# mims-harvard/GNNDelete

Measured on AMD Instinct MI355X. Metric: Del-op train iters/sec, higher is better.
Workload: dtype f32; 1 GPU; synth-collab GCN 2-layer, 5.0% IN edge deletion, full-graph Del step (both_layerwise, mse_mean); num_nodes=235868, in_dim=128, hidden_dim=128, out_dim=64, train_edges_undirected=2122296, df_edges=53057, sdf_edges=1602188, spmm_nnz=1838056, S1=178921, S2=188697, hip_graph=True, matrix_products=fp32 matrix instruction (v_mfma_f32_32x32x2_f32), parallelism=single, ranks_seen=1

## Files before the change

gnndelete_amd/_lib.py:

```python
import ctypes
import os
import re

_HERE = os.path.dirname(os.path.abspath(__file__))
LIB_PATH = os.environ.get('GNNDELETE_HIP_LIB') or os.path.join(_HERE, 'lib', 'libgnndelete_hip.so')
HEADER_PATH = os.path.join(os.path.dirname(_HERE), 'include', 'gnndelete_hip.h')

_i32, _i64, _f32, _f64, _p = ctypes.c_int32, ctypes.c_int64, ctypes.c_float, ctypes.c_double, ctypes.c_void_p

ABI_VERSION = 9

PROTOTYPES = {
    'gd_abi_version': (ctypes.c_int, []),
    'gd_last_error_string': (ctypes.c_char_p, []),
    'gd_build_source_hash': (ctypes.c_char_p, []),
    'gd_matrix_split': (ctypes.c_int, []),
    'gd_set_matrix_split': (ctypes.c_int, [ctypes.c_int]),
    'gd_csr_from_coo_workspace': (_i64, [_i32, _i64]),
    'gd_csr_from_coo': (ctypes.c_int, [_p, _p, _i64, _i32, _p, _p, _p, _p, _p, _i64, _p]),
    'gd_gcn_norm_f32': (ctypes.c_int, [_p, _p, _i32, _p, _p]),
    'gd_spmm_csr_f32': (ctypes.c_int, [_p, _p, _p, _p, _i64, _p, _i64, _p, _f32, _i32, _i32, _p]),
    'gd_spmm_csr_balanced_f32': (ctypes.c_int, [_p, _i32, _p, _i32, _p, _p, _p, _i64, _p, _i64, _p, _f32, _p, _p, _i32,
                                                _i32, _i32, _p, _p]),
    'gd_spmm_csr_onepass_f32': (ctypes.c_int, [_p, _i32, _p, _p, _p, _i64, _p, _i64, _p, _f32, _p, _i32, _i32, _i32, _p, _p]),
    'gd_spmm_csr_onepass_wide_f32': (ctypes.c_int, [_p, _i32, _p, _p, _p, _i64, _p, _i64, _p, _f32, _p, _i32, _i32, _i32, _p, _p]),
    'gd_rows_gemm_wgrad_reduce_f32': (ctypes.c_int, [_p, _i32, _i32, _i32, _p, _i32, _p, _p, _p, _p, _f64, _f64, _f64, _f64, _p]),
    'gd_step_tail_f32': (ctypes.c_int, [_p, _i32, _i32, _i32, _p, _p, _p, _p, _p, _i32, _i32, _i32, _p, _p, _p, _p, _f64, _f64, _f64, _f64,
                                        _p, _i32, _p, _i32, _p, _i32, _p, _p, _p, _p]),
    'gd_step_tail_parts_f32': (ctypes.c_int, [_p, _i32, _i32, _i32, _p, _p, _p, _p, _p, _i32, _i32, _i32, _p, _p, _p, _p, _f64, _f64, _f64, _f64,
                                        _p, _i32, _p, _i32, _p, _i32, _p, _p, _p, _p]),
    'gd_rgcn_conv_f32': (ctypes.c_int, [_p, _p, _p, _p, _p, _p, _i64, _i32, _p, _i32, _i32, _p, _i64, _i32, _i32, _p]),
    'gd_rowpair_loss_f32': (ctypes.c_int, [_i32, _p, _i64, _p, _p, _i64, _p, _i32, _i32, _p, _p, _i64, _p]),
    'gd_random_walk': (ctypes.c_int, [_p, _p, _i32, _p, _i32, _i32, ctypes.c_uint64, _p, _p]),
    'gd_negative_edges': (ctypes.c_int, [_p, _i64, _i64, ctypes.c_uint64, _p, _i64, _p, _i64, _p]),
    'gd_rank_counts_f32': (ctypes.c_int, [_p, _i64, _p, _i64, _p, _p, _p]),
    'gd_subset_rank_workspace': (_i64, [_i64, _i64]),
    'gd_subset_rank_metrics': (ctypes.c_int, [_p, _p, _p, _p, _p, _i64, _i64, _i64, _i64, _i64, _p, _p, _p, _i64, _p]),
    'gd_subset_rank_metrics_drawn': (ctypes.c_int, [_p, _p, _p, _p, ctypes.c_uint64, ctypes.c_uint64, _i64, _i64, _i64, _i64, _p, _p, _p, _i64, _p]),
    'gd_subset_draw': (ctypes.c_int, [ctypes.c_uint64, ctypes.c_uint64, _i64, _i64, _i64, _p, _i64, _p]),
    'gd_rgcn_tile_kl': (ctypes.c_int32, [_i32, _i32, _i32, _i32]),
    'gd_rgcn_pack_weight_f32': (ctypes.c_int, [_p, _i32, _i32, _i32, _i32, _i32, _p, _p]),
    'gd_rgcn_wave_covers': (ctypes.c_int32, [_i32, _i32, _i32]),
    'gd_rgcn_wave_conv_f32': (ctypes.c_int, [_p, _i32, _i32, _p, _i32, _p, _p, _p, _p, _i64, _i32, _p, _i32, _p, _i64, _i32, _i32, _i32, _p]),
    'gd_rgcn_tile_conv_f32': (ctypes.c_int, [_p, _p, _p, _p, _p, _p, _p, _i32, _p, _i64, _i32, _p, _i32, _i32, _p, _i64, _i32,
                                             _i32, _p, _p, _i32, _p, _p]),
    'gd_rgcn_mean_f32': (ctypes.c_int, [_p, _p, _p, _i64, _p, _i64, _i32, _i32, _i32, _p]),
    'gd_gat_aggregate_f32': (ctypes.c_int, [_p, _p, _p, _p, _p, _i64, _p, _i64, _p, _p, _f32, _i32, _i32, _p]),
    'gd_gat_aggregate_bwd_f32': (ctypes.c_int, [_p, _p, _p, _p, _p, _p, _p, _p, _p, _i64, _p, _i64, _p, _i64,
                                                _p, _p, _p, _f32, _i32, _i32, _p]),
    'gd_gat_balanced_scratch': (_i64, [_i32, _i32]),
    'gd_gat_aggregate_balanced_f32': (ctypes.c_int, [_p, _i32, _p, _i32, _i32, _p, _p, _p, _p, _i64, _p, _i64, _p, _p, _p,
                                                     _p, _f32, _i32, _i32, _i32, _p]),
    'gd_gat_edge_grads_balanced_f32': (ctypes.c_int, [_p, _i32, _p, _i32, _p, _p, _p, _p, _p, _p, _i64, _p, _i64, _p,
                                                      _p, _p, _p, _f32, _i32, _i32, _p, _p]),
    'gd_row_dots_f32': (ctypes.c_int, [_p, _i64, _i32, _i32, _p, _p, _p, _p, _p]),
    'gd_gat_transpose_edges_f32': (ctypes.c_int, [_p, _p, _p, _i32, _p, _p, _p]),
    'gd_rank1_add2_f32': (ctypes.c_int, [_p, _i64, _i32, _i32, _p, _p, _p, _p, _p]),
    'gd_segment_sum_f32': (ctypes.c_int, [_p, _p, _p, _i32, _p, _p]),
# ... 166 lines not shown
```

gnndelete_amd/csrc/spmm.hip:

```cpp
#include <stdlib.h>
#include <string.h>

#include "common.h"
#include "tail_jobs.h"

namespace gd {

template <int LPR, int VPL, bool MEAN>
__global__ __launch_bounds__(256) void spmm_vec_kernel(const int32_t* __restrict__ rowptr,
                                                       const int32_t* __restrict__ col,
                                                       const float* __restrict__ val,
                                                       const float* __restrict__ x, int64_t ldx,
                                                       float* __restrict__ y, int64_t ldy,
                                                       const float* __restrict__ bias, float self_coef,
                                                       int32_t n_rows, int32_t x_rows_mod, int32_t d4) {
  constexpr int G = kWave / LPR;
  const int lane = threadIdx.x & 63;
  const int row = blockIdx.x * 4 + (threadIdx.x >> 6);
  if (row >= n_rows) return;
  const int g = lane / LPR;
  const int li = lane % LPR;
  const int start = rowptr[row];
  const int end = rowptr[row + 1];

// ... 482 lines not shown
          acc = f4_fma(wj[2], xv[2], f4_fma(wj[1], xv[1], f4_fma(wj[0], xv[0], acc)));
        }
        base += kWave;
        if (base >= d0.z) break;
        const int k2 = min(base + lane, nnz - 1);
        c_cur = colt[k2];
        w_raw = val ? val[k2] : 1.0f;
      }
      acc = f4_group_sum<16>(acc);
      const int wave = threadIdx.x >> 6;
      if (g == 0) grp_red[wave][li] = acc;
      __syncthreads();
      if (wave == 0 && g == 0) {
        float4 o = f4_add(f4_add(f4_add(grp_red[0][li], grp_red[1][li]), grp_red[2][li]), grp_red[3][li]);
        if (self_coef != 0.0f)
          o = f4_fma(self_coef, *reinterpret_cast<const float4*>(reinterpret_cast<const char*>(xs) + (__umul24((uint32_t)row, pitch_b) + lo)), o);
        if (bias) o = f4_add(o, bias_s[li]);
        *reinterpret_cast<float4*>(reinterpret_cast<char*>(y) + (__umul24((uint32_t)row, pitch_y) + lo)) = o;
      }
      __syncthreads();
    }
    d0 = d1;
    d1 = d2;
  }
}

__global__ __launch_bounds__(256) __attribute__((amdgpu_waves_per_eu(8, 8))) void spmm_wide_kernel(
    const int4* __restrict__ items, int32_t n_items, const int32_t* __restrict__ xcd_bounds, const int32_t* __restrict__ colt,
    const float* __restrict__ val, const float* __restrict__ x, int64_t ldx, float* __restrict__ y, int64_t ldy,
    const float* __restrict__ bias, float self_coef, const float* __restrict__ xs, int32_t nnz) {
  spmm_wide_body(items, n_items, xcd_bounds, colt, val, x, ldx, y, ldy, bias, self_coef, xs, nnz, blockIdx.x, gridDim.x);
}

__global__ __launch_bounds__(256) __attribute__((amdgpu_waves_per_eu(8, 8))) void spmm_wide_hosted_kernel(
    const int4* __restrict__ items, int32_t n_items, const int32_t* __restrict__ xcd_bounds, const int32_t* __restrict__ colt,
    const float* __restrict__ val, const float* __restrict__ x, int64_t ldx, float* __restrict__ y, int64_t ldy,
    const float* __restrict__ bias, float self_coef, const float* __restrict__ xs, int32_t nnz, TailHost host) {
  if (blockIdx.x < (uint32_t)host.nh) {
    tail_host_block(host, (int)blockIdx.x);
    return;
  }
  spmm_wide_body(items, n_items, xcd_bounds, colt, val, x, ldx, y, ldy, bias, self_coef, xs, nnz, blockIdx.x - host.nh, gridDim.x - host.nh);
}

__global__ __launch_bounds__(256) void spmm_fixup_kernel(const int4* __restrict__ split, int32_t n_split,
                                                         const float* __restrict__ scratch,
                                                         const float* __restrict__ x, int64_t ldx,
                                                         float* __restrict__ y, int64_t ldy,
                                                         const float* __restrict__ bias, float self_coef,
                                                         int32_t d4) {
  const int lane = threadIdx.x & 63;
  const int i = blockIdx.x * 4 + (threadIdx.x >> 6);
  if (i >= n_split) return;
  const int4 sp = split[i];
  const int row = sp.x, slot0 = sp.y, n = sp.z;
  for (int vec = lane; vec < d4; vec += kWave) {
    float4 o = f4_zero();
    const float4* sp4 = reinterpret_cast<const float4*>(scratch + (int64_t)slot0 * d4 * 4) + vec;
    int s = 0;
    for (; s + 4 <= n; s += 4) {
      const float4 p0 = sp4[(int64_t)s * d4], p1 = sp4[(int64_t)(s + 1) * d4], p2 = sp4[(int64_t)(s + 2) * d4],
                   p3 = sp4[(int64_t)(s + 3) * d4];
      o = f4_add(f4_add(f4_add(f4_add(o, p0), p1), p2), p3);
    }
    for (; s < n; ++s) o = f4_add(o, sp4[(int64_t)s * d4]);
    if (self_coef != 0.0f) o = f4_fma(self_coef, reinterpret_cast<const float4*>(x + (int64_t)row * ldx)[vec], o);
// ... 186 lines not shown
  const float* xs = x_self ? x_self : x;
  GD_REQUIRE(aligned16(xs) && xs != y, GD_E_ALIGN, "gd_spmm_csr_balanced_f32: bad x_self");
  float* scratch_arg = scratch ? scratch : reinterpret_cast<float*>(const_cast<int32_t*>(items));
  int rc = launch_persist(items, n_items, col, val, x, ldx, y, ldy, bias, self_coef, xs, scratch_arg, d, nnz, x_rows,
                          xcd_bounds, s);
  if (rc || n_split == 0) return rc;
  hipLaunchKernelGGL(spmm_fixup_kernel, dim3((n_split + 3) / 4), dim3(256), 0, s, reinterpret_cast<const int4*>(split),
                     n_split, scratch, xs, ldx, y, ldy, bias, self_coef, d4);
  return launched("spmm_fixup");
}

extern "C" int gd_spmm_csr_onepass_f32(const int32_t* items, int32_t n_items, const int32_t* col, const float* val,
                                       const float* x, int64_t ldx, float* y, int64_t ldy, const float* bias,
                                       float self_coef, const float* x_self, int32_t d, int32_t nnz, int32_t x_rows,
                                       const int32_t* xcd_bounds, void* stream) {
  using namespace gd;
  GD_REQUIRE(col && x && y && xcd_bounds && (items || n_items == 0), GD_E_NULL, "gd_spmm_csr_onepass_f32: null pointer");
  GD_REQUIRE(n_items >= 0 && n_items % 4 == 0 && d > 0 && d % 4 == 0 && d <= 1024 && ldx % 4 == 0 && ldy % 4 == 0, GD_E_DIM,
             "gd_spmm_csr_onepass_f32: d=%d must be a multiple of 4 (<=1024) with 16-byte row strides, n_items a multiple of 4", d);
  GD_REQUIRE(aligned16(x) && aligned16(y) && aligned16(items) && (!bias || aligned16(bias)), GD_E_ALIGN,
             "gd_spmm_csr_onepass_f32: unaligned pointer");
  GD_REQUIRE(x != y, GD_E_DIM, "gd_spmm_csr_onepass_f32: x and y must not alias");
  if (n_items == 0) return GD_OK;
  GD_REQUIRE(nnz > 0, GD_E_DIM, "gd_spmm_csr_onepass_f32: items over an index array without entries (nnz=%d)", nnz);
  const float* xs = x_self ? x_self : x;
  GD_REQUIRE(aligned16(xs) && xs != y, GD_E_ALIGN, "gd_spmm_csr_onepass_f32: bad x_self");
  return launch_persist(items, n_items, col, val, x, ldx, y, ldy, bias, self_coef, xs, nullptr, d, nnz, x_rows,
                        xcd_bounds, (hipStream_t)stream);
}

namespace gd {
static int launch_wide(const char* name, const int32_t* items, int32_t n_items, const int32_t* col_tagged, const float* val, const float* x,
                       int64_t ldx, float* y, int64_t ldy, const float* bias, float self_coef, const float* x_self, int32_t d,
                       int32_t nnz, int32_t x_rows, const int32_t* xcd_bounds, const TailHost* host, void* stream) {
  GD_REQUIRE(col_tagged && x && y && xcd_bounds && (items || n_items == 0), GD_E_NULL, "%s: null pointer", name);
  GD_REQUIRE(n_items >= 0 && n_items % 4 == 0 && d == 64 && ldx % 4 == 0 && ldy % 4 == 0 && ldx >= d && ldy >= d, GD_E_DIM,
             "%s: d must be 64 (got %d) with 16-byte row strides, n_items a multiple of 4", name, d);
  GD_REQUIRE(aligned16(x) && aligned16(y) && aligned16(items) && (!bias || aligned16(bias)), GD_E_ALIGN, "%s: unaligned pointer", name);
  GD_REQUIRE(x != y, GD_E_DIM, "%s: x and y must not alias", name);
  GD_REQUIRE(x_rows > 0 && x_rows < (1 << 24) && ldx * 4 < (1 << 24) && ldy * 4 < (1 << 24) &&
                 (int64_t)x_rows * ldx * 4 < (1ll << 32) && (int64_t)x_rows * ldy * 4 < (1ll << 32), GD_E_DIM,
             "%s: x and y must be smaller than 4 GiB with row ids and pitches below 2^24", name);
  GD_REQUIRE(!host || n_items > 0, GD_E_DIM, "%s: the tail's jobs need a launch to ride on (n_items = 0)", name);
  if (n_items == 0) return GD_OK;
  GD_REQUIRE(nnz > 0, GD_E_DIM, "%s: items over an index array without entries (nnz=%d)", name, nnz);
  const float* xs = x_self ? x_self : x;
  GD_REQUIRE(aligned16(xs) && xs != y, GD_E_ALIGN, "%s: bad x_self", name);
  const char* e = getenv("GD_SPMM_GRID_CAP");
  const int cap_env = e ? atoi(e) : 0;
  const int cap = cap_env > 0 ? cap_env : GD_SPMM_WIDE_GRID_CAP;
  int nblk = (n_items + 3) / 4;
  if (nblk > cap) nblk = cap;
  nblk = (nblk + 7) / 8 * 8;
  if (host) {
    hipLaunchKernelGGL(spmm_wide_hosted_kernel, dim3(host->nh + nblk), dim3(256), 0, (hipStream_t)stream,
                       reinterpret_cast<const int4*>(items), n_items, xcd_bounds, col_tagged, val, x, ldx, y, ldy, bias, self_coef, xs, nnz,
                       *host);
    return launched("spmm_wide_hosted");
  }
  hipLaunchKernelGGL(spmm_wide_kernel, dim3(nblk), dim3(256), 0, (hipStream_t)stream, reinterpret_cast<const int4*>(items), n_items,
                     xcd_bounds, col_tagged, val, x, ldx, y, ldy, bias, self_coef, xs, nnz);
  return launched("spmm_wide");
}
}

extern "C" int gd_spmm_csr_onepass_wide_f32(const int32_t* items, int32_t n_items, const int32_t* col_tagged, const float* val,
                                            const float* x, int64_t ldx, float* y, int64_t ldy, const float* bias,
                                            float self_coef, const float* x_self, int32_t d, int32_t nnz, int32_t x_rows,
                                            const int32_t* xcd_bounds, void* stream) {
  return gd::launch_wide("gd_spmm_csr_onepass_wide_f32", items, n_items, col_tagged, val, x, ldx, y, ldy, bias, self_coef, x_self, d, nnz,
                         x_rows, xcd_bounds, nullptr, stream);
}

extern "C" int gd_spmm_csr_onepass_wide_hosted_f32(
    const int32_t* items, int32_t n_items, const int32_t* col_tagged, const float* val, const float* x, int64_t ldx, float* y, int64_t ldy,
    const float* bias, float self_coef, const float* x_self, int32_t d, int32_t nnz, int32_t x_rows, const int32_t* xcd_bounds,
    const float* partials1_t, const float* colsum1, int32_t n_part1, int32_t d1, const float* w1, const float* w1_t, const float* b1,
    float* dw1, float* param1, float* exp_avg1, float* exp_avg_sq1, float* w_fold, float* bias_fold, const float* partials2,
    int32_t n_part2, int32_t d2, int32_t accumulate2, float* dw2, float* param2, float* exp_avg2, float* exp_avg_sq2, double lr,
    double beta1, double beta2, double eps, const float* loss_partials1, int32_t n1, const float* loss_partials2, int32_t n2, float* hist,
    int32_t capacity, int32_t* pos, int32_t* iter, int32_t* arrive, void* stream) {
  using namespace gd;
  const char* name = "gd_spmm_csr_onepass_wide_hosted_f32";
  GD_REQUIRE(n_part1 >= 0 && n_part2 >= 0 && n_part1 + n_part2 > 0, GD_E_DIM,
             "%s: a hosted launch carries job 1, job 2 or both (partial counts %d, %d)", name, n_part1, n_part2);
  GD_REQUIRE(iter, GD_E_NULL, "%s: null iteration counter", name);
  TailHost h{};
  h.lr = lr; h.beta1 = beta1; h.beta2 = beta2; h.eps = eps;
  h.fin = TailFin{loss_partials1, n1, loss_partials2, n2, hist, capacity, pos, iter, arrive};
  if (n_part1 > 0) {
    GD_REQUIRE(partials1_t && colsum1 && w1 && w1_t && b1 && dw1 && param1 && exp_avg1 && exp_avg_sq1 && w_fold && bias_fold, GD_E_NULL,
               "%s: null pointer of job 1", name);
    GD_REQUIRE(d1 == 128, GD_E_DIM, "%s: the folded layer-1 job is 128 wide (d1=%d)", name, d1);
    GD_REQUIRE(aligned16(partials1_t), GD_E_ALIGN, "%s: unaligned partials of job 1", name);
    h.j1 = TailJob{partials1_t, n_part1, d1 * d1, 0, dw1, param1, exp_avg1, exp_avg_sq1};
    h.fo = TailFold1{colsum1, w1, b1, w_fold, bias_fold};
    h.w1t = w1_t;
    h.n1b = 128;
  }
  if (n_part2 > 0) {
    GD_REQUIRE(partials2 && dw2 && param2 && exp_avg2 && exp_avg_sq2, GD_E_NULL, "%s: null pointer of job 2", name);
    GD_REQUIRE(hist && pos && arrive && capacity > 0 && n1 >= 0 && n2 >= 0 && (n1 == 0 || loss_partials1) && (n2 == 0 || loss_partials2),
               GD_E_NULL, "%s: null bookkeeping pointer", name);
    GD_REQUIRE(d2 > 0 && d2 % 4 == 0 && d2 <= 128, GD_E_DIM, "%s: d2=%d must be a multiple of 4, at most 128", name, d2);
// ... 39 lines not shown
```

gnndelete_amd/engine.py:

```python
import os
import warnings
from typing import NamedTuple

import torch

from . import _lib, ops
from ._lib import check, ptr, stream_ptr
from .capture import capture_iterations
from .graph import graph_for
from .nn import GATConv, GCNConv, GINConv, RGCNConv, SAGEConv

LOSS_TYPES = ('both_all', 'both_layerwise', 'only2_layerwise', 'only2_all', 'only1')


class StepFacts(NamedTuple):
    mode: str
    loss_type: str
    family: str
    h: int
    o: int
    s1: int
    s2: int
    folded1: bool
    n_rows1: int
# ... 663 lines not shown
        if idx is not None or self._mfma_weight(weight):
            return ops.rows_gemm(x, idx, weight, trans_w=True, const_w=True, relu_in=relu_in, out=out)
        if ops.mfma_out_width(out_f):
            xin = torch.relu(x) if relu_in else x
            return ops.gemm_wide(xin, ops._const_weight(weight, True)[0], const_x=not relu_in, const_w=True)
        if in_f <= 1024:
            return ops.rows_gemm(x, None, weight, trans_w=True, const_w=True, relu_in=relu_in)
        raise NotImplementedError(f'NodeembEngine: a {in_f} -> {out_f} Linear has no kernel (inputs above 1,024 floats need an output '
                                  'width in {32, 64, 96, 128}); there is no vendor-BLAS fallback')

    def _linear_relu_z1(self, weight, idx=None, out=None):
        if not self._split1:
            return self._linear(self.z1, weight, relu_in=True, idx=idx, out=out)
        if self._chain_expl:
            assert idx is None
            return ops.rows_gemm_select_chain(self._a1, self._idx1c, self._w1, self._b1, self.pre1, self.z1, self.idx1, weight, out=out)
        if idx is not None or self._mfma_weight(weight):
            return ops.rows_gemm_select(self.pre1, self.z1, self._sel1, weight, trans_w=True, const_w=True, relu_in=True,
                                        out=out, idx=idx)
        z = torch.where(self._sel1.bool()[:, None], self.z1, self.pre1)
        return self._linear(z, weight, relu_in=True)

    def _layer1_rows(self, weight):
        if self._rows_only and self._split1 and self._mfma_weight(weight):
            return self.idx2, self._t1buf, self._plan2
        return None, None, None

    def _conv1_forward(self):
        c = self.model.conv1
        g = self.graph
        if self._mode == 'rgcn':
            self._rgcn_conv(c, self.x, self.pre1, 0)
        elif self._mode == 'gcn' and self._fold1:
            self._spmm(False, g.val, self.x, self._a1, None, 0.0, plan=self._plan2 if self._rows_only else None)
            if self._idx1c.numel() and not self._chain_expl:
                ops.rows_gemm(self._a1, self._idx1c, self._w1, trans_w=True, const_w=True, bias=self._b1, out=self.pre1)
        elif self._mode == 'gcn':
            idx, out, plan = self._layer1_rows(c.lin.weight)
            self._spmm(False, g.val, self._linear(self.x, c.lin.weight, idx=idx, out=out), self.pre1, c.bias, 0.0, plan=plan)
        elif self._mode == 'gin':
            lin = c.nn
            if lin.out_features <= lin.in_features:
                idx, out, plan = self._layer1_rows(lin.weight)
                self._spmm(False, None, self._linear(self.x, lin.weight, idx=idx, out=out), self.pre1, lin.bias, 1.0 + c.eps, plan=plan)
            else:
                agg = torch.empty_like(self.x)
                self._spmm(False, None, self.x, agg, None, 1.0 + c.eps)
                ops.rows_gemm(agg, None, lin.weight, trans_w=True, const_w=True, bias=lin.bias, out=self.pre1)
        elif self._mode == 'sage':
            idx, out, plan = self._layer1_rows(c.lin_l.weight)
            t_l = self._linear(self.x, c.lin_l.weight, idx=idx, out=out)
            if (idx is None and self._mfma_weight(c.lin_r.weight)
                    and ops.rows_gemm_accumulate_ok(self.n, c.lin_r.weight.shape[1], c.lin_r.weight.shape[0])
                    and not self.knobs.sage_root_in_spmm):
                self._spmm(False, g.val, t_l, self.pre1, c.lin_l.bias, 0.0)
                ops.rows_gemm_accumulate_(self.pre1, self.x, None, c.lin_r.weight, trans_w=True, const_w=True)
            else:
                t_r = self._linear(self.x, c.lin_r.weight, idx=idx, out=None if idx is None else self._t1rbuf)
                self._spmm(False, g.val, t_l, self.pre1, c.lin_l.bias, 1.0, x_self=t_r, plan=plan)
        else:
            wsrc = c.lin_src.weight
            idx, out, _ = self._layer1_rows(wsrc)
            if idx is None and self._gat_dots and ops.rows_gemm_dots_ok(wsrc.shape[1], wsrc.shape[0], self.n):
                h1, a_src, a_dst = ops.rows_gemm_dots(self.x, wsrc, c.att_src, c.att_dst, const_w=True)
            else:
                h1 = self._linear(self.x, wsrc, idx=idx, out=out)
                a_src, a_dst = ops.row_dots(h1, c.att_src, c.att_dst)
# ... 65 lines not shown
                       plan=self._plan_t1 if self._rows_only else None)
            dt2, w2 = self.dcat, self._w2cat
        elif self._mode in ('gcn', 'gin'):
            chain = self._chain1
            if self._rows_only:
                dt2, plan = self._dt2buf, self._plan_t1
            else:
                dt2, plan = (self._dt2_keep if chain else torch.empty(self.n, self.o, dtype=torch.float32, device=self.x.device)), None
            if self._mode == 'gcn':
                self._spmm(True, g.val_t, self.dz2, dt2, None, 0.0, plan=plan, host=self._tail_host(2))
                w2 = c.lin.weight
            else:
                self._spmm(True, None, self.dz2, dt2, None, 1.0 + c.eps, plan=plan)
                w2 = c.nn.weight
            if chain:
                return
        else:
            chain = self._chain1
            dt2, da_s, da_d = ops.gat_backward_raw(g, self._h2, self._a_src, self._a_dst, self._rowmax, self._rowsum,
                                                   self.dz2, c.negative_slope,
                                                   plan=self._plan2 if self._rows_only else None,
                                                   plan_t=self._plan_t1 if self._rows_only else None,
                                                   bufs=self._gat_bufs if chain else None)
            if chain:
                return
            w2 = c.lin_src.weight
            if self._mfma_weight(w2) and not self.knobs.no_gat_rank1_epilogue:
                ops.rows_gemm(dt2, self.idx1, w2, trans_w=False, out=self.dh, gate_bits=self.z1_pos,
                              rank1=(da_s, self._gat_r1[0], da_d, self._gat_r1[1]))
                return
            ops.rank1_add2_(dt2, da_s, c.att_src, da_d, c.att_dst)
        ops.rows_gemm(dt2, self.idx1, w2, trans_w=False, out=self.dh, gate_bits=self.z1_pos)

    def _spmm(self, transposed, val, x, y, bias, self_coef, x_self=None, plan=None, host=None):
        g = self.graph
        if transposed:
            ops._spmm_raw(g.rowptr_t, g.col_t, val, x, bias, self_coef, self.n, plan or g.plan_t, out=y, x_self=x_self, host=host)
        else:
            ops._spmm_raw(g.rowptr, g.col, val, x, bias, self_coef, self.n, plan or g.plan, out=y, x_self=x_self, host=host)

    def step_stages(self):
        if not (self._fold1 and self._fold2 and self._chain1 and self._tail and not self._rows_only):
            return None
        stages = ['spmm1'] + ([] if self._chain_expl else ['pre1_rest']) + ['del1_loss_wgrad1', 't2', 'spmm2', 'del2_loss_bwd', 'spmm2_t']
        return stages + ([] if self._tail_hosted else ['tail'])

    def _loss_partials(self):
        p1, n1 = ((self._lp1, self._lp1_blocks + (self.t1.outside_blocks() if self._out1 else 0)) if self._fuse_loss1
                  else (self.t1.partials, self.t1.n_partial_blocks()))
        p2, n2 = ((self._lp2, self._lp2_blocks + (self.t2.outside_blocks() if self._out2 else 0)) if self._fuse_l2
                  else (self.t2.partials, self.t2.n_partial_blocks()))
        return p1, n1, p2, n2

    def _tail_host(self, job):
        if not self._tail_hosted:
            return None
        a1, a2 = self.adam1, self.adam2
        p1, n1, p2, n2 = self._loss_partials()
        return (ptr(self.ws1), ptr(self._cs1), self._lp1_blocks if job == 1 else 0, self.h, ptr(self._w1), ptr(self._w1t), ptr(self._b1),
                ptr(self.g1), ptr(a1.param), ptr(a1.m), ptr(a1.v), ptr(self._wf), ptr(self._bf),
                ptr(self.ws2), self._lp2_blocks if job == 2 else 0, self.o, self._tail_acc[1], ptr(self.g2), ptr(a2.param), ptr(a2.m),
                ptr(a2.v), a1.lr, a1.betas[0], a1.betas[1], a1.eps,
                ptr(p1), n1, ptr(p2), n2, ptr(self.hist), self.hist.shape[0], ptr(self.hist_pos), ptr(self.iter_ctr), ptr(self._arrive))

    def _wgrad(self, a_compact, g, g_idx, n_sel, out, accumulate, ws, adam=None, g_add=None, a_idx=None):
        d_a, d_b = a_compact.shape[1], g.shape[1]
        if adam is not None:
            adam.applied += 1
        if adam is None or self._tail:
            if adam is not None:
                self._tail_acc[0 if adam is self.adam1 else 1] = int(accumulate)
            check(_lib.lib().gd_rows_gemm_wgrad_f32(ptr(a_compact), a_compact.stride(0), ptr(a_idx), ptr(g), g.stride(0),
# ... 264 lines not shown
```

gnndelete_amd/graph.py:

```python
import os

import torch

from . import _lib


CHUNK = 64
WIDE_ROWS = 16
WIDE_VISIT_COST = 48


class SplitPlan:

    def __init__(self, rowptr, chunk=CHUNK, row_range=None, rows=None):
        dev = rowptr.device
        rpl = rowptr.long()
        if rows is not None:
            ids = rows.long()
        else:
            lo, hi = (0, rowptr.numel() - 1) if row_range is None else row_range
            ids = torch.arange(lo, hi, device=dev)
        r_start, r_end = rpl[ids], rpl[ids + 1]
        self._outside = None
        if rows is not None or row_range is not None:
            self._outside = torch.ones(rowptr.numel() - 1, dtype=torch.bool, device=dev)
            self._outside[ids] = False
        n = ids.numel()
        deg = r_end - r_start
        pieces = torch.clamp((deg + chunk - 1) // chunk, min=1)
        first = torch.cumsum(pieces, 0) - pieces
        row = torch.repeat_interleave(torch.arange(n, device=dev), pieces)
        k = torch.arange(row.numel(), device=dev) - first[row]
        start = r_start[row] + k * chunk
        end = torch.minimum(r_end[row], start + chunk)
        is_split = pieces[row] > 1
        slot = torch.where(is_split, torch.cumsum(is_split, 0) - 1, torch.full_like(row, -1))
        self.items = torch.stack([ids[row], start, end, slot], 1).to(torch.int32).contiguous()
        self.n_items = int(row.numel())
        srows = (pieces > 1).nonzero().flatten()
        split_pieces = torch.where(pieces > 1, pieces, torch.zeros_like(pieces))
        slot0 = (torch.cumsum(split_pieces, 0) - split_pieces)[srows]
        self.split = torch.stack([ids[srows], slot0, pieces[srows], torch.zeros_like(srows)], 1).to(torch.int32).contiguous()
# ... 216 lines not shown
                total += 4 * int(big.numel())
            rest = (pk <= 4).nonzero().flatten() + lo
            if rest.numel():
                is_hub = pieces[rest] > 1
                op = opener[rest] & ~is_hub
                opens = op.long()
                light_run = torch.cumsum(opens, 0)
                hub_pos = is_hub.nonzero().flatten()
                prev = torch.cat([light_run.new_zeros(1), light_run[hub_pos][:-1]]) if hub_pos.numel() else light_run.new_zeros(0)
                pad = (-(light_run[hub_pos] - prev)) % 4
                slots = opens.clone()
                slots[hub_pos] = 4 + pad
                off = torch.cumsum(slots, 0) - slots
                m = int(slots.sum())
                blk = pad_item.expand(m, 4).clone()
                o = rest[op]
                if o.numel():
                    blk[off[op]] = torch.stack([ids[o], r_start[o], r_end[nxt[o] - 1], -(16 + nxt[o] - o - 1)], 1)
                if hub_pos.numel():
                    first = off[hub_pos] + pad
                    blk[(first[:, None] + q4[None, :]).reshape(-1)] = members(rest[hub_pos])
                parts.append(blk)
                total += m
            tail = (-total) % 4
            if tail:
                parts.append(pad_item.expand(tail, 4))
                total += tail
            bounds.append(total)
        items = torch.cat(parts, 0).to(torch.int32).contiguous() if parts else torch.zeros(0, 4, dtype=torch.int32, device=dev)
        assert all(b % 4 == 0 for b in bounds) and total % 4 == 0, bounds
        hit = (items, total, torch.tensor(bounds, dtype=torch.int32, device=dev), tags)
        self._onepass[key] = hit
        return hit

    def rows_outside(self):
        return self._outside

    def scratch_flat(self, tag, n_floats, device):
        buf = self._scratch.get(tag)
        if buf is None or buf.numel() < n_floats:
            buf = torch.empty(max(int(n_floats), 4), dtype=torch.float32, device=device)
            self._scratch[tag] = buf
        return buf

    def scratch(self, d, device):
        if self.n_slots == 0:
            return None
        buf = self._scratch.get(d)
        if buf is None:
            buf = torch.empty(self.n_slots, d, dtype=torch.float32, device=device)
            self._scratch[d] = buf
        return buf


class CSRGraph:

    def __init__(self, n, rowptr, col, val, rowptr_t, col_t, val_t, perm_t, mode):
        self.n, self.mode = n, mode
        self.rowptr, self.col, self.val = rowptr, col, val
        self.rowptr_t, self.col_t, self.val_t, self.perm_t = rowptr_t, col_t, val_t, perm_t
        self.nnz = int(col.shape[0])
        self.plan = SplitPlan(rowptr)
        self.plan_t = SplitPlan(rowptr_t)

    @property
    def device(self):
# ... 442 lines not shown
```

gnndelete_amd/ops.py:

```python
import os

import torch

from . import _lib
from ._lib import check, ptr, stream_ptr


def matrix_split():
    return _lib.lib().gd_matrix_split()


def set_matrix_split(n_products):
    _lib.check(_lib.lib().gd_set_matrix_split(int(n_products)), 'gd_set_matrix_split')


def _f32_rows(t):
    if t.device.type != 'cuda':
        raise _lib.GnnDeleteHipError('gnndelete_amd ops need CUDA(HIP) tensors; got a CPU tensor (no CPU fallback)')
    if t.dtype != torch.float32:
        t = t.float()
    if t.dim() != 2 or t.stride(1) != 1 or t.stride(0) < t.shape[1] or (t.stride(0) % 4 and t.shape[1] % 4 == 0):
        t = t.contiguous()
    return t




def spmm_wide_form(d, x_rows, ld_x, ld_y, env=None):
    env = os.environ if env is None else env
    return bool(d == 64 and ld_x % 4 == 0 and x_rows < (1 << 24) and ld_x * 4 < (1 << 24) and ld_y * 4 < (1 << 24)
                and x_rows * ld_x * 4 < (1 << 32) and x_rows * ld_y * 4 < (1 << 32) and env.get('GD_SPMM_TWO_LAUNCH') != '1'
                and env.get('GD_SPMM_MULTIROW') != '0' and not env.get('GD_SPMM_D64_FORM'))


def _no_host(host):
    if host is not None:
        raise _lib.GnnDeleteHipError('the step tail can only ride on the wide 64-float aggregation (gd_spmm_csr_onepass_wide_hosted_f32)')


def _spmm_raw(rowptr, col, val, x, bias, self_coef, n_rows, plan=None, out=None, x_self=None, wide=True, host=None):
    d = x.shape[1]
    if x_self is not None:
        assert plan is not None and x_self.stride(0) == x.stride(0) and x_self.shape[1] == d
    y = out if out is not None else torch.empty(n_rows, d, dtype=torch.float32, device=x.device)
    if int(col.shape[0]) == 0:
        _no_host(host)
        xs = x if x_self is None else x_self
        r = xs[:n_rows] * float(self_coef) if self_coef != 0.0 else torch.zeros(n_rows, d, dtype=torch.float32, device=x.device)
        if bias is not None:
            r = r + bias
        outside = plan.rows_outside() if plan is not None else None
        if outside is None:
            y[:n_rows].copy_(r)
        else:
            y[:n_rows][~outside] = r[~outside]
        return y
    if (plan is not None and d % 4 == 0 and d <= 1024 and x.stride(0) % 4 == 0 and x.data_ptr() % 16 == 0
            and os.environ.get('GD_SPMM_TWO_LAUNCH') != '1'):
        x_rows = max(int(x.shape[0]), int(y.shape[0]))
        if wide and spmm_wide_form(d, x_rows, x.stride(0), y.stride(0)):
            items, n_items, bounds, tags = plan.onepass_wide(d)
            args = (ptr(items), n_items, ptr(_wide_col(plan, col, tags)), ptr(val), ptr(x), x.stride(0), ptr(y), y.stride(0), ptr(bias),
                    float(self_coef), ptr(x_self), d, int(col.shape[0]), x_rows, ptr(bounds))
            if host is not None:
                check(_lib.lib().gd_spmm_csr_onepass_wide_hosted_f32(*args, *host, stream_ptr(x.device)), 'gd_spmm_csr_onepass_wide_hosted_f32')
                return y
            check(_lib.lib().gd_spmm_csr_onepass_wide_f32(*args, stream_ptr(x.device)), 'gd_spmm_csr_onepass_wide_f32')
            return y
        _no_host(host)
        items, n_items, bounds = plan.onepass(d)
        check(_lib.lib().gd_spmm_csr_onepass_f32(ptr(items), n_items, ptr(col), ptr(val), ptr(x), x.stride(0), ptr(y),
                                                 y.stride(0), ptr(bias), float(self_coef), ptr(x_self), d, int(col.shape[0]),
                                                 max(int(x.shape[0]), int(y.shape[0])), ptr(bounds), stream_ptr(x.device)),
              'gd_spmm_csr_onepass_f32')
        return y
    _no_host(host)
    if plan is not None and d % 4 == 0 and d <= 1024 and x.stride(0) % 4 == 0 and x.data_ptr() % 16 == 0:
        scratch = plan.scratch(d, x.device)
        check(_lib.lib().gd_spmm_csr_balanced_f32(ptr(plan.items), plan.n_items, ptr(plan.split), plan.n_split,
                                                  ptr(col), ptr(val), ptr(x), x.stride(0), ptr(y), y.stride(0),
                                                  ptr(bias), float(self_coef), ptr(x_self), ptr(scratch), d, int(col.shape[0]),
                                                  max(int(x.shape[0]), int(y.shape[0])), ptr(plan.xcd_bounds(d)),
                                                  stream_ptr(x.device)),
              'gd_spmm_csr_balanced_f32')
        return y
    assert x_self is None, 'x_self needs the balanced kernel (d % 4 == 0, 16-byte aligned rows)'
    check(_lib.lib().gd_spmm_csr_f32(ptr(rowptr), ptr(col), ptr(val), ptr(x), x.stride(0), ptr(y), y.stride(0),
                                     ptr(bias), float(self_coef), n_rows, d, stream_ptr(x.device)),
          'gd_spmm_csr_f32')
    return y


class _SpMM(torch.autograd.Function):

    @staticmethod
    def forward(ctx, x, bias, graph, self_coef):
        x = _f32_rows(x)
        ctx.graph, ctx.self_coef = graph, self_coef
        ctx.has_bias = bias is not None
        return _spmm_raw(graph.rowptr, graph.col, graph.val, x, bias, self_coef, graph.n, graph.plan)

    @staticmethod
# ... 913 lines not shown
```

include/gnndelete_hip.h:

```cpp
#ifndef GNNDELETE_HIP_H
#define GNNDELETE_HIP_H

#include <stdint.h>

#ifdef __cplusplus
extern "C" {
#endif

#define GD_ABI_VERSION 9

enum {
  GD_OK = 0,
  GD_E_NULL = 1,
  GD_E_DIM = 2,
  GD_E_ALIGN = 3,
  GD_E_WORKSPACE = 4
};

int gd_abi_version(void);
const char* gd_last_error_string(void);
const char* gd_build_source_hash(void);

#define GD_MATRIX_SPLIT_DEFAULT 0
int gd_matrix_split(void);
int gd_set_matrix_split(int n_products);


int64_t gd_csr_from_coo_workspace(int32_t n_nodes, int64_t n_edges);
int gd_csr_from_coo(const int64_t* src, const int64_t* dst, int64_t n_edges, int32_t n_nodes, int32_t* rowptr,
                    int32_t* col, int32_t* order, int32_t* status, void* workspace, int64_t workspace_bytes,
                    void* stream);


int gd_gcn_norm_f32(const int32_t* rowptr, const int32_t* col, int32_t n_rows, float* val, void* stream);

int gd_spmm_csr_f32(const int32_t* rowptr, const int32_t* col, const float* val,
                    const float* x, int64_t ldx, float* y, int64_t ldy, const float* bias,
                    float self_coef, int32_t n_rows, int32_t d, void* stream);

int gd_spmm_csr_balanced_f32(const int32_t* items, int32_t n_items, const int32_t* split, int32_t n_split,
                             const int32_t* col, const float* val, const float* x, int64_t ldx,
                             float* y, int64_t ldy, const float* bias, float self_coef,
                             const float* x_self, float* scratch, int32_t d, int32_t nnz, int32_t x_rows,
                             const int32_t* xcd_bounds, void* stream);

int gd_spmm_csr_onepass_f32(const int32_t* items, int32_t n_items, const int32_t* col, const float* val,
                            const float* x, int64_t ldx, float* y, int64_t ldy, const float* bias, float self_coef,
                            const float* x_self, int32_t d, int32_t nnz, int32_t x_rows, const int32_t* xcd_bounds,
                            void* stream);

int gd_spmm_csr_onepass_wide_f32(const int32_t* items, int32_t n_items, const int32_t* col_tagged, const float* val,
                                 const float* x, int64_t ldx, float* y, int64_t ldy, const float* bias, float self_coef,
                                 const float* x_self, int32_t d, int32_t nnz, int32_t x_rows, const int32_t* xcd_bounds,
                                 void* stream);

int gd_spmm_csr_onepass_aux_f32(const int32_t* items, int32_t n_items, const int32_t* col, const int32_t* perm, const float* aux,
                                const float* x, int64_t ldx, float* y, int64_t ldy, float* aux_sum, int32_t d, int32_t nnz,
                                int32_t x_rows, const int32_t* xcd_bounds, void* stream);


int gd_rgcn_mean_f32(const int32_t* rowptr, const int32_t* col, const float* x, int64_t ldx,
                     float* y, int64_t ldy, int32_t n_rel, int32_t n_rows, int32_t d, void* stream);

int gd_gat_aggregate_f32(const int32_t* rowptr, const int32_t* col, const float* a_src, const float* a_dst,
                         const float* h, int64_t ldh, float* y, int64_t ldy, const float* bias,
                         float* alpha_out, float slope, int32_t n_rows, int32_t d, void* stream);

int gd_gat_aggregate_bwd_f32(const int32_t* rowptr, const int32_t* col, const float* alpha,
                             const int32_t* rowptr_t, const int32_t* col_t, const int32_t* perm_t,
                             const float* a_src, const float* a_dst, const float* h, int64_t ldh,
                             const float* dy, int64_t lddy, float* dh, int64_t lddh,
                             float* da_src, float* da_dst, float* de, float slope,
                             int32_t n_rows, int32_t d, void* stream);

int64_t gd_gat_balanced_scratch(int32_t n_slots, int32_t d);
int gd_gat_aggregate_balanced_f32(const int32_t* items, int32_t n_items, const int32_t* split, int32_t n_split,
                                  int32_t n_slots, const int32_t* col, const float* a_src, const float* a_dst,
                                  const float* h, int64_t ldh, float* y, int64_t ldy, const float* bias,
                                  float* rowmax, float* rowsum, float* scratch, float slope,
                                  int32_t d, int32_t nnz, int32_t h_rows , void* stream);
int gd_gat_edge_grads_balanced_f32(const int32_t* items, int32_t n_items, const int32_t* split, int32_t n_split,
                                   const int32_t* col, const float* a_src, const float* a_dst,
                                   const float* rowmax, const float* rowsum, const float* h, int64_t ldh,
                                   const float* dy, int64_t lddy, float* ade, float* da_dst,
                                   float* t_row, float* scratch, float slope, int32_t d, int32_t nnz, const int32_t* xcd_bounds,
        void* stream);

// ... 361 lines not shown
```

Before: 2166 iters/s.

## Add MFMA-based wide SpMM kernel for 128-wide features in layer-1 aggregation

Adds a 128-column variant of the wide one-pass SpMM that packs 16 destination rows per wave and accumulates neighbour contributions with 16x16x4 fp32 MFMA instructions. Heavy rows fall back to a per-block reduction path. The layer-1 folded GCN aggregation (d=128) now uses this kernel, reusing the 64-wide row tagging and item plan. It aims to replace the generic one-pass vector kernel with a batched-row matrix-instruction path, at the cost of wasted MFMA lanes on sparse rows and higher register pressure.

```diff
diff --git a/gnndelete_amd/_lib.py b/gnndelete_amd/_lib.py
--- a/gnndelete_amd/_lib.py
+++ b/gnndelete_amd/_lib.py
@@ -24,6 +24,7 @@
                                                 _i32, _i32, _p, _p]),
     'gd_spmm_csr_onepass_f32': (ctypes.c_int, [_p, _i32, _p, _p, _p, _i64, _p, _i64, _p, _f32, _p, _i32, _i32, _i32, _p, _p]),
     'gd_spmm_csr_onepass_wide_f32': (ctypes.c_int, [_p, _i32, _p, _p, _p, _i64, _p, _i64, _p, _f32, _p, _i32, _i32, _i32, _p, _p]),
+    'gd_spmm_csr_onepass_wide128_f32': (ctypes.c_int, [_p, _i32, _p, _p, _p, _i64, _p, _i64, _p, _f32, _p, _i32, _i32, _i32, _p, _p]),
     'gd_rows_gemm_wgrad_reduce_f32': (ctypes.c_int, [_p, _i32, _i32, _i32, _p, _i32, _p, _p, _p, _p, _f64, _f64, _f64, _f64, _p]),
     'gd_step_tail_f32': (ctypes.c_int, [_p, _i32, _i32, _i32, _p, _p, _p, _p, _p, _i32, _i32, _i32, _p, _p, _p, _p, _f64, _f64, _f64, _f64,
                                         _p, _i32, _p, _i32, _p, _i32, _p, _p, _p, _p]),
diff --git a/gnndelete_amd/csrc/spmm.hip b/gnndelete_amd/csrc/spmm.hip
--- a/gnndelete_amd/csrc/spmm.hip
+++ b/gnndelete_amd/csrc/spmm.hip
@@ -538,6 +538,202 @@
   spmm_wide_body(items, n_items, xcd_bounds, colt, val, x, ldx, y, ldy, bias, self_coef, xs, nnz, blockIdx.x, gridDim.x);
 }
 
+template <int UM>
+__device__ __forceinline__ void spmm_wide128_body(
+    const int4* __restrict__ items, int32_t n_items, const int32_t* __restrict__ xcd_bounds, const int32_t* __restrict__ colt,
+    const float* __restrict__ val, const float* __restrict__ x, int64_t ldx, float* __restrict__ y, int64_t ldy,
+    const float* __restrict__ bias, float self_coef, const float* __restrict__ xs, int32_t nnz, uint32_t bid, uint32_t nblk) {
+  constexpr int kXcd = 8, U = 4, H = 2;
+  constexpr int kSrcMask = (1 << 24) - 1;
+  constexpr int LH = 16 * H, GSH = 1;
+  const int lane = threadIdx.x & 63;
+  const int g = lane >> 4, li = lane & 15;
+  const int xcd = bid % kXcd;
+  const int stride = (nblk / kXcd) * 4;
+  const int wx = (bid / kXcd) * 4 + (threadIdx.x >> 6);
+  const int i0 = xcd_bounds[xcd], i1 = xcd_bounds[xcd + 1];
+  if ((i0 | i1) & 3) __builtin_trap();
+  const uint32_t lo = 16u * (uint32_t)li;
+  const uint32_t pitch_b = (uint32_t)ldx * 4u, pitch_y = (uint32_t)ldy * 4u;
+  const char* xb = reinterpret_cast<const char*>(x);
+
+  int i = __builtin_amdgcn_readfirstlane(i0 + wx);
+  if (i >= i1) return;
+  int4 d0 = items[i], d1 = items[min(i + stride, i1 - 1)];
+  int kk = min(d0.y + lane, nnz - 1);
+  int c = colt[kk];
+  float w = val ? val[kk] : 1.0f;
+  __shared__ float4 grp_red[4][LH];
+  __shared__ float4 bias_s[LH];
+  if (threadIdx.x < LH) bias_s[threadIdx.x] = bias ? reinterpret_cast<const float4*>(bias)[threadIdx.x] : f4_zero();
+  __syncthreads();
+  for (; i < i1; i += stride) {
+    const int row = d0.x, slot = d0.w;
+    const int c_now = c;
+    const float w_now = w;
+    const int4 d2 = items[min(i + 2 * stride, i1 - 1)];
+    kk = min(d1.y + lane, nnz - 1);
+    c = colt[kk];
+    w = val ? val[kk] : 1.0f;
+    if (slot != -2) {
+      const int nr = -slot - 15;
+      const int cnt = d0.z - d0.y;
+      const float w_cur = lane < cnt ? w_now : 0.f;
+      const int trips = (cnt + 3) >> 2;
+      const int last4 = 4 * cnt - 4, end4 = 4 * cnt;
+      f32x4_t a[H][4];
+#pragma unroll
+      for (int h = 0; h < H; ++h) {
+        const float4 bv = bias_s[16 * h + li];
+        a[h][0] = f32x4_t{bv.x, bv.x, bv.x, bv.x};
+        a[h][1] = f32x4_t{bv.y, bv.y, bv.y, bv.y};
+        a[h][2] = f32x4_t{bv.z, bv.z, bv.z, bv.z};
+        a[h][3] = f32x4_t{bv.w, bv.w, bv.w, bv.w};
+      }
+      auto fetch = [&](int t, float4(&xv)[H], float& av) {
+        const int j4 = 16 * t + 4 * g;
+        const int cs = __builtin_amdgcn_ds_bpermute(min(j4, last4), c_now);
+        const float wj = __int_as_float(__builtin_amdgcn_ds_bpermute(min(j4, end4), __float_as_int(w_cur)));
+        av = ((uint32_t)cs >> 24) == (uint32_t)li ? wj : 0.f;
+        const uint32_t ro = __umul24((uint32_t)(cs & kSrcMask), pitch_b);
+#pragma unroll
+        for (int h = 0; h < H; ++h) xv[h] = *reinterpret_cast<const float4*>(xb + (ro + lo) + 256 * h);
+      };
+      auto mma = [&](float av, const float4(&xv)[H]) {
+#pragma unroll
+        for (int h = 0; h < H; ++h) {
+          a[h][0] = __builtin_amdgcn_mfma_f32_16x16x4f32(av, xv[h].x, a[h][0], 0, 0, 0);
+          a[h][1] = __builtin_amdgcn_mfma_f32_16x16x4f32(av, xv[h].y, a[h][1], 0, 0, 0);
+          a[h][2] = __builtin_amdgcn_mfma_f32_16x16x4f32(av, xv[h].z, a[h][2], 0, 0, 0);
+          a[h][3] = __builtin_amdgcn_mfma_f32_16x16x4f32(av, xv[h].w, a[h][3], 0, 0, 0);
+        }
+      };
+      int t0 = 0;
+      for (; t0 + UM <= trips; t0 += UM) {
+        float4 xv[UM][H];
+        float av[UM];
+#pragma unroll
+        for (int u = 0; u < UM; ++u) fetch(t0 + u, xv[u], av[u]);
+        __builtin_amdgcn_sched_barrier(0);
+#pragma unroll
+        for (int u = 0; u < UM; ++u) mma(av[u], xv[u]);
+      }
+      const int rem = trips - t0;
+      if (rem == 1) {
+        float4 xv[1][H];
+        float av;
+        fetch(t0, xv[0], av);
+        mma(av, xv[0]);
+      } else if (UM > 2 && rem == 2) {
+        float4 xv[2][H];
+        float av[2];
+        fetch(t0, xv[0], av[0]);
+        fetch(t0 + 1, xv[1], av[1]);
+        mma(av[0], xv[0]);
+        mma(av[1], xv[1]);
+      } else if (UM > 2 && rem == 3) {
+        float4 xv[3][H];
+        float av[3];
+        fetch(t0, xv[0], av[0]);
+        fetch(t0 + 1, xv[1], av[1]);
+        fetch(t0 + 2, xv[2], av[2]);
+        mma(av[0], xv[0]);
+        mma(av[1], xv[1]);
+        mma(av[2], xv[2]);
+      }
+      const uint32_t r0 = (uint32_t)(row + 4 * g);
+#pragma unroll
+      for (int j = 0; j < 4; ++j) {
+        if (4 * g + j < nr) {
+#pragma unroll
+          for (int h = 0; h < H; ++h) {
+            float4 o = make_float4(a[h][0][j], a[h][1][j], a[h][2][j], a[h][3][j]);
+            if (self_coef != 0.0f)
+              o = f4_fma(self_coef, *reinterpret_cast<const float4*>(reinterpret_cast<const char*>(xs) + (__umul24(r0 + j, pitch_b) + lo) + 256 * h), o);
+            *reinterpret_cast<float4*>(reinterpret_cast<char*>(y) + (__umul24(r0 + j, pitch_y) + lo) + 256 * h) = o;
+          }
+        }
+      }
+    } else {
+      const int gh = lane >> (6 - GSH), lh = lane & (LH - 1);
+      const uint32_t loh = 16u * (uint32_t)lh;
+      int base = d0.y;
+      int c_cur = c_now;
+      float w_raw = w_now;
+      float4 acc = f4_zero();
+      for (;;) {
+        const int cnt = min(kWave, d0.z - base);
+        const float w_cur = lane < cnt ? w_raw : 0.f;
+        const int trips = (cnt + (1 << GSH) - 1) >> GSH;
+        const int last4 = 4 * cnt - 4, end4 = 4 * cnt;
+        auto fetch = [&](int t, float4& xv, float& wj) {
+          const int j4 = (4 << GSH) * t + 4 * gh;
+          const int cs = __builtin_amdgcn_ds_bpermute(min(j4, last4), c_cur);
+          wj = __int_as_float(__builtin_amdgcn_ds_bpermute(min(j4, end4), __float_as_int(w_cur)));
+          const uint32_t ro = __umul24((uint32_t)(cs & kSrcMask), pitch_b);
+          xv = *reinterpret_cast<const float4*>(xb + (ro + loh));
+        };
+        int t0 = 0;
+        for (; t0 + U <= trips; t0 += U) {
+          float4 xv[U];
+          float wj[U];
+#pragma unroll
+          for (int u = 0; u < U; ++u) fetch(t0 + u, xv[u], wj[u]);
+#pragma unroll
+          for (int u = 0; u < U; ++u) acc = f4_fma(wj[u], xv[u], acc);
+        }
+        const int rem = trips - t0;
+        if (rem == 1) {
+          float4 xv;
+          float wj;
+          fetch(t0, xv, wj);
+          acc = f4_fma(wj, xv, acc);
+        } else if (rem == 2) {
+          float4 xv[2];
+          float wj[2];
+          fetch(t0, xv[0], wj[0]);
+          fetch(t0 + 1, xv[1], wj[1]);
+          acc = f4_fma(wj[1], xv[1], f4_fma(wj[0], xv[0], acc));
+        } else if (rem == 3) {
+          float4 xv[3];
+          float wj[3];
+          fetch(t0, xv[0], wj[0]);
+          fetch(t0 + 1, xv[1], wj[1]);
+          fetch(t0 + 2, xv[2], wj[2]);
+          acc = f4_fma(wj[2], xv[2], f4_fma(wj[1], xv[1], f4_fma(wj[0], xv[0], acc)));
+        }
+        base += kWave;
+        if (base >= d0.z) break;
+        const int k2 = min(base + lane, nnz - 1);
+        c_cur = colt[k2];
+        w_raw = val ? val[k2] : 1.0f;
+      }
+      acc = f4_group_sum<LH>(acc);
+      const int wave = threadIdx.x >> 6;
+      if (gh == 0) grp_red[wave][lh] = acc;
+      __syncthreads();
+      if (wave == 0 && gh == 0) {
+        float4 o = f4_add(f4_add(f4_add(grp_red[0][lh], grp_red[1][lh]), grp_red[2][lh]), grp_red[3][lh]);
+        if (self_coef != 0.0f)
+          o = f4_fma(self_coef, *reinterpret_cast<const float4*>(reinterpret_cast<const char*>(xs) + (__umul24((uint32_t)row, pitch_b) + loh)), o);
+        if (bias) o = f4_add(o, bias_s[lh]);
+        *reinterpret_cast<float4*>(reinterpret_cast<char*>(y) + (__umul24((uint32_t)row, pitch_y) + loh)) = o;
+      }
+      __syncthreads();
+    }
+    d0 = d1;
+    d1 = d2;
+  }
+}
+
+template <int UM, int WAVES>
+__global__ __launch_bounds__(256) __attribute__((amdgpu_waves_per_eu(WAVES, WAVES))) void spmm_wide128_kernel(
+    const int4* __restrict__ items, int32_t n_items, const int32_t* __restrict__ xcd_bounds, const int32_t* __restrict__ colt,
+    const float* __restrict__ val, const float* __restrict__ x, int64_t ldx, float* __restrict__ y, int64_t ldy,
+    const float* __restrict__ bias, float self_coef, const float* __restrict__ xs, int32_t nnz) {
+  spmm_wide128_body<UM>(items, n_items, xcd_bounds, colt, val, x, ldx, y, ldy, bias, self_coef, xs, nnz, blockIdx.x, gridDim.x);
+}
+
 __global__ __launch_bounds__(256) __attribute__((amdgpu_waves_per_eu(8, 8))) void spmm_wide_hosted_kernel(
     const int4* __restrict__ items, int32_t n_items, const int32_t* __restrict__ xcd_bounds, const int32_t* __restrict__ colt,
     const float* __restrict__ val, const float* __restrict__ x, int64_t ldx, float* __restrict__ y, int64_t ldy,
@@ -790,10 +986,10 @@
 namespace gd {
 static int launch_wide(const char* name, const int32_t* items, int32_t n_items, const int32_t* col_tagged, const float* val, const float* x,
                        int64_t ldx, float* y, int64_t ldy, const float* bias, float self_coef, const float* x_self, int32_t d,
-                       int32_t nnz, int32_t x_rows, const int32_t* xcd_bounds, const TailHost* host, void* stream) {
+                       int32_t nnz, int32_t x_rows, const int32_t* xcd_bounds, const TailHost* host, void* stream, int32_t width = 64) {
   GD_REQUIRE(col_tagged && x && y && xcd_bounds && (items || n_items == 0), GD_E_NULL, "%s: null pointer", name);
-  GD_REQUIRE(n_items >= 0 && n_items % 4 == 0 && d == 64 && ldx % 4 == 0 && ldy % 4 == 0 && ldx >= d && ldy >= d, GD_E_DIM,
-             "%s: d must be 64 (got %d) with 16-byte row strides, n_items a multiple of 4", name, d);
+  GD_REQUIRE(n_items >= 0 && n_items % 4 == 0 && d == width && ldx % 4 == 0 && ldy % 4 == 0 && ldx >= d && ldy >= d, GD_E_DIM,
+             "%s: d must be %d (got %d) with 16-byte row strides, n_items a multiple of 4", name, width, d);
   GD_REQUIRE(aligned16(x) && aligned16(y) && aligned16(items) && (!bias || aligned16(bias)), GD_E_ALIGN, "%s: unaligned pointer", name);
   GD_REQUIRE(x != y, GD_E_DIM, "%s: x and y must not alias", name);
   GD_REQUIRE(x_rows > 0 && x_rows < (1 << 24) && ldx * 4 < (1 << 24) && ldy * 4 < (1 << 24) &&
@@ -810,6 +1006,16 @@
   int nblk = (n_items + 3) / 4;
   if (nblk > cap) nblk = cap;
   nblk = (nblk + 7) / 8 * 8;
+  if (width == 128) {
+    const char* t = getenv("GD_SPMM_WIDE128_TRIPS");
+    if (t && atoi(t) == 4)
+      hipLaunchKernelGGL((spmm_wide128_kernel<4, 5>), dim3(nblk), dim3(256), 0, (hipStream_t)stream, reinterpret_cast<const int4*>(items), n_items,
+                         xcd_bounds, col_tagged, val, x, ldx, y, ldy, bias, self_coef, xs, nnz);
+    else
+      hipLaunchKernelGGL((spmm_wide128_kernel<2, 7>), dim3(nblk), dim3(256), 0, (hipStream_t)stream, reinterpret_cast<const int4*>(items), n_items,
+                         xcd_bounds, col_tagged, val, x, ldx, y, ldy, bias, self_coef, xs, nnz);
+    return launched("spmm_wide128");
+  }
   if (host) {
     hipLaunchKernelGGL(spmm_wide_hosted_kernel, dim3(host->nh + nblk), dim3(256), 0, (hipStream_t)stream,
                        reinterpret_cast<const int4*>(items), n_items, xcd_bounds, col_tagged, val, x, ldx, y, ldy, bias, self_coef, xs, nnz,
@@ -828,6 +1034,14 @@
                                             const int32_t* xcd_bounds, void* stream) {
   return gd::launch_wide("gd_spmm_csr_onepass_wide_f32", items, n_items, col_tagged, val, x, ldx, y, ldy, bias, self_coef, x_self, d, nnz,
                          x_rows, xcd_bounds, nullptr, stream);
+}
+
+extern "C" int gd_spmm_csr_onepass_wide128_f32(const int32_t* items, int32_t n_items, const int32_t* col_tagged, const float* val,
+                                               const float* x, int64_t ldx, float* y, int64_t ldy, const float* bias,
+                                               float self_coef, const float* x_self, int32_t d, int32_t nnz, int32_t x_rows,
+                                               const int32_t* xcd_bounds, void* stream) {
+  return gd::launch_wide("gd_spmm_csr_onepass_wide128_f32", items, n_items, col_tagged, val, x, ldx, y, ldy, bias, self_coef, x_self, d,
+                         nnz, x_rows, xcd_bounds, nullptr, stream, 128);
 }
 
 extern "C" int gd_spmm_csr_onepass_wide_hosted_f32(
diff --git a/gnndelete_amd/engine.py b/gnndelete_amd/engine.py
--- a/gnndelete_amd/engine.py
+++ b/gnndelete_amd/engine.py
@@ -719,7 +719,7 @@
         if self._mode == 'rgcn':
             self._rgcn_conv(c, self.x, self.pre1, 0)
         elif self._mode == 'gcn' and self._fold1:
-            self._spmm(False, g.val, self.x, self._a1, None, 0.0, plan=self._plan2 if self._rows_only else None)
+            self._spmm(False, g.val, self.x, self._a1, None, 0.0, plan=self._plan2 if self._rows_only else None, wide128=True)
             if self._idx1c.numel() and not self._chain_expl:
                 ops.rows_gemm(self._a1, self._idx1c, self._w1, trans_w=True, const_w=True, bias=self._b1, out=self.pre1)
         elif self._mode == 'gcn':
@@ -851,12 +851,12 @@
             ops.rank1_add2_(dt2, da_s, c.att_src, da_d, c.att_dst)
         ops.rows_gemm(dt2, self.idx1, w2, trans_w=False, out=self.dh, gate_bits=self.z1_pos)
 
-    def _spmm(self, transposed, val, x, y, bias, self_coef, x_self=None, plan=None, host=None):
+    def _spmm(self, transposed, val, x, y, bias, self_coef, x_self=None, plan=None, host=None, wide128=False):
         g = self.graph
         if transposed:
-            ops._spmm_raw(g.rowptr_t, g.col_t, val, x, bias, self_coef, self.n, plan or g.plan_t, out=y, x_self=x_self, host=host)
+            ops._spmm_raw(g.rowptr_t, g.col_t, val, x, bias, self_coef, self.n, plan or g.plan_t, out=y, x_self=x_self, host=host, wide128=wide128)
         else:
-            ops._spmm_raw(g.rowptr, g.col, val, x, bias, self_coef, self.n, plan or g.plan, out=y, x_self=x_self, host=host)
+            ops._spmm_raw(g.rowptr, g.col, val, x, bias, self_coef, self.n, plan or g.plan, out=y, x_self=x_self, host=host, wide128=wide128)
 
     def step_stages(self):
         if not (self._fold1 and self._fold2 and self._chain1 and self._tail and not self._rows_only):
diff --git a/gnndelete_amd/graph.py b/gnndelete_amd/graph.py
--- a/gnndelete_amd/graph.py
+++ b/gnndelete_amd/graph.py
@@ -8,6 +8,9 @@
 CHUNK = 64
 WIDE_ROWS = 16
 WIDE_VISIT_COST = 48
+
+
+WIDE128_VISIT_COST = 48
 
 
 class SplitPlan:
@@ -290,6 +293,11 @@
         hit = (items, total, torch.tensor(bounds, dtype=torch.int32, device=dev), tags)
         self._onepass[key] = hit
         return hit
+
+    def onepass_wide128(self, visit_cost=None):
+        a = WIDE128_VISIT_COST if visit_cost is None else int(visit_cost)
+        items, n, bounds, _ = self.onepass_wide(64, visit_cost=a)
+        return items, n, bounds, self.onepass_wide(64)[3]
 
     def rows_outside(self):
         return self._outside
diff --git a/gnndelete_amd/ops.py b/gnndelete_amd/ops.py
--- a/gnndelete_amd/ops.py
+++ b/gnndelete_amd/ops.py
@@ -33,12 +33,19 @@
                 and env.get('GD_SPMM_MULTIROW') != '0' and not env.get('GD_SPMM_D64_FORM'))
 
 
+def spmm_wide128_form(d, x_rows, ld_x, ld_y, env=None):
+    env = os.environ if env is None else env
+    return bool(d == 128 and ld_x % 4 == 0 and x_rows < (1 << 24) and ld_x * 4 < (1 << 24) and ld_y * 4 < (1 << 24)
+                and x_rows * ld_x * 4 < (1 << 32) and x_rows * ld_y * 4 < (1 << 32) and env.get('GD_SPMM_TWO_LAUNCH') != '1'
+                and env.get('GD_SPMM_MULTIROW') != '0' and env.get('GD_SPMM_D128_FORM') != 'items')
+
+
 def _no_host(host):
     if host is not None:
         raise _lib.GnnDeleteHipError('the step tail can only ride on the wide 64-float aggregation (gd_spmm_csr_onepass_wide_hosted_f32)')
 
 
-def _spmm_raw(rowptr, col, val, x, bias, self_coef, n_rows, plan=None, out=None, x_self=None, wide=True, host=None):
+def _spmm_raw(rowptr, col, val, x, bias, self_coef, n_rows, plan=None, out=None, x_self=None, wide=True, host=None, wide128=False):
     d = x.shape[1]
     if x_self is not None:
         assert plan is not None and x_self.stride(0) == x.stride(0) and x_self.shape[1] == d
@@ -68,6 +75,12 @@
             check(_lib.lib().gd_spmm_csr_onepass_wide_f32(*args, stream_ptr(x.device)), 'gd_spmm_csr_onepass_wide_f32')
             return y
         _no_host(host)
+        if wide and (wide128 or os.environ.get('GD_SPMM_D128_FORM') == 'wide') and spmm_wide128_form(d, x_rows, x.stride(0), y.stride(0)):
+            items, n_items, bounds, tags = plan.onepass_wide128()
+            check(_lib.lib().gd_spmm_csr_onepass_wide128_f32(ptr(items), n_items, ptr(_wide_col(plan, col, tags)), ptr(val), ptr(x), x.stride(0),
+                                                             ptr(y), y.stride(0), ptr(bias), float(self_coef), ptr(x_self), d, int(col.shape[0]),
+                                                             x_rows, ptr(bounds), stream_ptr(x.device)), 'gd_spmm_csr_onepass_wide128_f32')
+            return y
         items, n_items, bounds = plan.onepass(d)
         check(_lib.lib().gd_spmm_csr_onepass_f32(ptr(items), n_items, ptr(col), ptr(val), ptr(x), x.stride(0), ptr(y),
                                                  y.stride(0), ptr(bias), float(self_coef), ptr(x_self), d, int(col.shape[0]),
diff --git a/include/gnndelete_hip.h b/include/gnndelete_hip.h
--- a/include/gnndelete_hip.h
+++ b/include/gnndelete_hip.h
@@ -53,6 +53,11 @@
                                  const float* x, int64_t ldx, float* y, int64_t ldy, const float* bias, float self_coef,
                                  const float* x_self, int32_t d, int32_t nnz, int32_t x_rows, const int32_t* xcd_bounds,
                                  void* stream);
+
+int gd_spmm_csr_onepass_wide128_f32(const int32_t* items, int32_t n_items, const int32_t* col_tagged, const float* val,
+                                    const float* x, int64_t ldx, float* y, int64_t ldy, const float* bias, float self_coef,
+                                    const float* x_self, int32_t d, int32_t nnz, int32_t x_rows, const int32_t* xcd_bounds,
+                                    void* stream);
 
 int gd_spmm_csr_onepass_aux_f32(const int32_t* items, int32_t n_items, const int32_t* col, const int32_t* perm, const float* aux,
                                 const float* x, int64_t ldx, float* y, int64_t ldy, float* aux_sum, int32_t d, int32_t nnz,
```

After: 2206 iters/s (median of 6 runs). +1.9%, better.
